# Grid2op/grid2op

Hardware: AMD Instinct MI355X
Metric: env steps/sec (batched DoNothing) (higher is better)
Workload: dtype f64; 1 GPU; l2rpn_case14_sandbox AC Newton-Raphson DoNothing env.step, batch=4096 lanes per GPU; env=l2rpn_case14_sandbox, lanes_per_gpu=4096, total_lanes=4096, env_steps_per_launch=16, observations=every env step -> HBM, cascade=False, kernels=grid-specialised at run time (gpf_jit_enable), parallelism=static lane shards x1, no collective

## Files before the change

grid2op_amd/csrc/gridpf_sparse.hpp:

```cpp
#pragma once
#include <type_traits>
#include "gridpf_common.hpp"

namespace gpf {

struct StatOff {
  int n_dbl, n_int;
  int n_int_hot;
  int br_y, br_bdc, sub_vn_kv, shunt_fact, gen_min_q, gen_max_q;
  int line_vn, load_vn, gen_vn, sto_vn, shunt_vn;
  int line_ka;
  int gen_qmin_tot, gen_qmax_tot;
  int gen_cnt;
  int dc_inv;
  int line_or_pos, line_ex_pos, line_or_sub, line_ex_sub, br_slot, gen_pos, gen_sub, gen_slack, load_pos, load_sub, sto_pos,
      sto_sub, shunt_sub, pair_rc, up, prog;
  int pos_line;
};
#define GPF_STATOFF_INTS(X) X(n_dbl) X(n_int) X(n_int_hot) X(br_y) X(br_bdc) X(sub_vn_kv) X(shunt_fact) X(gen_min_q) X(gen_max_q) X(line_vn) X(load_vn) \
  X(gen_vn) X(sto_vn) X(shunt_vn) X(line_ka) X(gen_qmin_tot) X(gen_qmax_tot) X(gen_cnt) X(dc_inv) X(line_or_pos) X(line_ex_pos) X(line_or_sub) \
  X(line_ex_sub) X(br_slot) X(gen_pos) X(gen_sub) X(gen_slack) X(load_pos) X(load_sub) X(sto_pos) X(sto_sub) X(shunt_sub) X(pair_rc) X(up) X(prog) X(pos_line)
static_assert(sizeof(StatOff) == sizeof(int) * (0 GPF_STATOFF_INTS(GPF_COUNT_FIELD)), "GPF_STATOFF_INTS must list every field of StatOff");
template <class T, bool IN_LDS>
struct SP {
// ... 530 lines not shown
      const double* Al = A + (size_t)(w0 & 0xffffu) * B2 + r * BS;
      const double* bp = rhs + (size_t)p * BS;
      double acc = 0.0;
#pragma unroll
      for (int m = 0; m < BS; ++m) acc = fma(Al[m], bp[m], acc);
      atomicAdd(&rhs[(size_t)(w0 >> 16) * BS + r], -acc);
    }
    GPF_LSYNC();
  }
#ifdef GPF_TIMING
  const long long t_lu1 = __builtin_readcyclecounter();
#endif
  for (int lv = S.n_levels - 1; lv >= 0; --lv) {
    const int ent_off = prog[S.back_off + 2 * lv], n_ent = prog[S.back_off + 2 * lv + 1];
    for (int it = tid; it < n_ent * BS; it += GW) {
      const unsigned w = (unsigned)prog[ent_off + 2 * (it / BS)];
      const int p = prog[ent_off + 2 * (it / BS) + 1], r = it % BS;
      const double* Au = A + (size_t)(w & 0xffffu) * B2 + r * BS;
      const double* xj = rhs + (size_t)(w >> 16) * BS;
      double acc = 0.0;
#pragma unroll
      for (int m = 0; m < BS; ++m) acc = fma(Au[m], xj[m], acc);
      atomicAdd(&rhs[(size_t)p * BS + r], -acc);
    }
    GPF_LSYNC();
  }
#ifdef GPF_TIMING
  if (dbg) { dbg[0] = t_lu1 - t_lu0; dbg[1] = (long long)__builtin_readcyclecounter() - t_lu1; }
#endif
  return ok;
}

constexpr int GPF_WR_CAP_F = 6, GPF_WR_CAP_B = 2;
template <bool ON> struct FlatWords { };
template <> struct FlatWords<true> { unsigned f[2 * GPF_WR_CAP_F], b[2 * GPF_WR_CAP_B]; };
#ifdef GPF_NO_WORDS_RES
template <int NB, int IPW, int WPI> constexpr bool flat_words_ct() { return false; }
#else
template <int NB, int IPW, int WPI> constexpr bool flat_words_ct() { return NB == 1 && IPW > 1 && WPI == 1; }
#endif
__device__ __forceinline__ bool flat_words_fit(const FlatDev& F) { return F.n_fwd <= GPF_WR_CAP_F && F.n_back <= GPF_WR_CAP_B; }
template <int GW, class PP>
__device__ __forceinline__ void flat_words_load(FlatWords<false>&, const FlatDev&, PP, int) {}
template <int GW, class PP>
__device__ __forceinline__ void flat_words_load(FlatWords<true>& W, const FlatDev& F, PP prog, int tid) {
  const bool fit = flat_words_fit(F);
#pragma unroll
  for (int k = 0; k < GPF_WR_CAP_F; ++k) {
    const bool on_f = fit && k < F.n_fwd;
    W.f[2 * k] = on_f ? (unsigned)prog[2 * tid + 2 * GW * k] : 0xffffffffu;
    W.f[2 * k + 1] = on_f ? (unsigned)prog[2 * tid + 2 * GW * k + 1] : 0u;
  }
#pragma unroll
  for (int k = 0; k < GPF_WR_CAP_B; ++k) {
    const bool on_b = fit && k < F.n_back;
    W.b[2 * k] = on_b ? (unsigned)prog[F.back_off + 2 * tid + 2 * GW * k] : 0xffffffffu;
    W.b[2 * k + 1] = on_b ? (unsigned)prog[F.back_off + 2 * tid + 2 * GW * k + 1] : 0u;
  }
}

template <int GW, class PP = const int*, bool RES = false>
__device__ inline bool block_lu_flat(const FlatDev& F, PP prog, double* __restrict__ A, size_t HS, int tid, long long* dbg = nullptr,
                                     const FlatWords<RES>* W = nullptr) {
#ifdef GPF_TIMING
  const long long t_lu0 = __builtin_readcyclecounter();
#endif
  bool ok = true;
#ifdef GPF_PF2_IG
  constexpr bool PF2 = GPF_PF2_ON && (GW > WAVE || (GW <= 32 && !std::is_same<PP, const int*>::value));
#else
  constexpr bool PF2 = GPF_PF2_ON && GW > WAVE;
#endif
  char* const a0 = reinterpret_cast<char*>(A);
  char* const a1 = a0 + HS * 8;
#define FL_LD2(base, f) (*reinterpret_cast<const double2*>((base) + (f)))
#define FL_D(base, f) (reinterpret_cast<double*>((base) + (f)))
#ifdef GPF_TIMING
#define GPF_PASS_T(i_) do { if (dbg && tid == 0 && (i_) < GPF_NPASS_T) gpf_pass_t[(i_)] = (long long)__builtin_readcyclecounter(); } while (0)
#else
#define GPF_PASS_T(i_) do {} while (0)
#endif
  GPF_PASS_T(0);
  auto fwd_item = [&](const unsigned w0, const unsigned w1) {
    if (w0 != 0xffffffffu) {
      const unsigned fd = w0 & 0xffffu, fl = w0 >> 16, fu = w1 & 0xffffu, fp = w1 >> 16;
      const double2 dA = FL_LD2(a0, fp), dB = FL_LD2(a1, fp), lA = FL_LD2(a0, fl), lB = FL_LD2(a1, fl);
      const double2 uA = FL_LD2(a0, fu), uB = FL_LD2(a1, fu);
      const double rd = -fast_rcp(fma(dA.x, dB.y, -dA.y * dB.x));
      const double t00 = fma(lA.x, dB.y, -lA.y * dB.x), t01 = fma(lA.y, dA.x, -lA.x * dA.y);
      const double t10 = fma(lB.x, dB.y, -lB.y * dB.x), t11 = fma(lB.y, dA.x, -lB.x * dA.y);
      double* d0_ = FL_D(a0, fd);
      double* d1_ = FL_D(a1, fd);
      atomicAdd(&d0_[0], fma(t00, uA.x, t01 * uB.x) * rd);
      atomicAdd(&d1_[0], fma(t10, uA.x, t11 * uB.x) * rd);
      if (fd < (unsigned)F.rhs_field0) {
        atomicAdd(&d0_[1], fma(t00, uA.y, t01 * uB.y) * rd);
        atomicAdd(&d1_[1], fma(t10, uA.y, t11 * uB.y) * rd);
      }
    }
  };
#define GPF_WALK(n_, at0_, MASK_, NEXT_SOLO_, ITEM_, TB_, WR_, CAP_)                                                                                 \
  {                                                                                                                                \
    const unsigned solo_ = GW > WAVE ? (unsigned)(MASK_) : 0u;                                                                     \
    const int n_pass_ = (n_);                                                                                                      \
    auto step_ = [&](const unsigned a_, const unsigned b_, const int k) {                                                          \
      const bool so_ = GW > WAVE && k < 32 && ((solo_ >> (k & 31)) & 1u);                                                          \
      if (!so_ || tid < WAVE) ITEM_(a_, b_);                                                                                       \
      const bool sn_ = so_ && (k + 1 < n_pass_ ? (k + 1 < 32 && ((solo_ >> ((k + 1) & 31)) & 1u)) : (GW > WAVE && (NEXT_SOLO_)));  \
      if (sn_) { asm volatile("" ::: "memory"); __builtin_amdgcn_wave_barrier(); asm volatile("" ::: "memory"); }                 \
      else GPF_LSYNC();                                                                                                            \
      GPF_PASS_T((TB_) + k);                                                                                                       \
    };                                                                                                                             \
    if constexpr (RES) {                                   \
      _Pragma("unroll")                                                                                                            \
      for (int k = 0; k < (CAP_); ++k)                                                                                             \
        if (k < n_pass_) step_(W->WR_[2 * k], W->WR_[2 * k + 1], k);                                                               \
    } else {                                                                                                                       \
    int at = (at0_) + 2 * tid;                                                                                                     \
    unsigned p0 = (unsigned)prog[at], p1 = (unsigned)prog[at + 1];                                                                 \
    if (PF2) {                                                                                                                     \
      at += 2 * GW;                                                                                                                \
      unsigned q0 = (unsigned)prog[at], q1 = (unsigned)prog[at + 1], r0, r1;                                                       \
      for (int k = 0; k < n_pass_; k += 3) {                                                                                       \
        at += 2 * GW; r0 = (unsigned)prog[at]; r1 = (unsigned)prog[at + 1];                                                        \
        step_(p0, p1, k);                                                                                                          \
        if (k + 1 >= n_pass_) break;                                                                                               \
        at += 2 * GW; p0 = (unsigned)prog[at]; p1 = (unsigned)prog[at + 1];                                                        \
        step_(q0, q1, k + 1);                                                                                                      \
        if (k + 2 >= n_pass_) break;                                                                                               \
        at += 2 * GW; q0 = (unsigned)prog[at]; q1 = (unsigned)prog[at + 1];                                                        \
        step_(r0, r1, k + 2);                                                                                                      \
      }                                                                                                                            \
    } else {                                                                                                                       \
      for (int k = 0; k < n_pass_; ++k) {                                                                                          \
        at += 2 * GW;                                                                                                              \
        const unsigned n0 = (unsigned)prog[at], n1 = (unsigned)prog[at + 1];                           \
        step_(p0, p1, k);                                                                                                          \
        p0 = n0; p1 = n1;                                                                                                          \
      }                                                                                                                            \
    }                                                                                                                              \
    }                                                                                                                              \
  }
  GPF_WALK(F.n_fwd, 0, F.solo_fwd, F.n_back > 0 && (F.solo_back & 1), fwd_item, 1, f, GPF_WR_CAP_F)
#ifdef GPF_TIMING
  const long long t_lu1 = __builtin_readcyclecounter();
#endif
  auto back_item = [&](const unsigned w0, const unsigned w1) {
    if (w0 != 0xffffffffu) {
      const unsigned fu = w0 & 0xffffu, fj = w0 >> 16, fdj = fj - (unsigned)F.rhs_field0;
      const double2 uA = FL_LD2(a0, fu), uB = FL_LD2(a1, fu), dA = FL_LD2(a0, fdj), dB = FL_LD2(a1, fdj);
      const double s0 = *FL_D(a0, fj), s1 = *FL_D(a1, fj);
      const double rd = fast_rcp(fma(dA.x, dB.y, -dA.y * dB.x));
      const double x0 = fma(dB.y, s0, -dA.y * s1) * rd, x1 = fma(dA.x, s1, -dB.x * s0) * rd;
      atomicAdd(FL_D(a0, w1), -fma(uA.x, x0, uA.y * x1));
      atomicAdd(FL_D(a1, w1), -fma(uB.x, x0, uB.y * x1));
    }
  };
  GPF_WALK(F.n_back, F.back_off, F.solo_back, false, back_item, 1 + F.n_fwd, b, GPF_WR_CAP_B)
#ifdef GPF_TIMING
  if (dbg) { dbg[0] = t_lu1 - t_lu0; dbg[1] = (long long)__builtin_readcyclecounter() - t_lu1; }
#endif
  return ok;
}

template <int GW, bool FACTOR, bool COMPACT, class PP = const int*, bool RES = false>
__device__ inline bool scalar_lu_flat(const FlatDev& F, PP prog, double* __restrict__ A, double* __restrict__ fac, int tid,
                                      long long* dbg = nullptr, const FlatWords<RES>* W = nullptr) {
#ifdef GPF_TIMING
  const long long t_lu0 = __builtin_readcyclecounter();
#endif
  bool ok = true;
#ifdef GPF_PF2_IG
  constexpr bool PF2 = GPF_PF2_ON && (GW > WAVE || (GW <= 32 && !std::is_same<PP, const int*>::value));
#else
  constexpr bool PF2 = GPF_PF2_ON && GW > WAVE;
#endif
  char* const a0 = reinterpret_cast<char*>(A);
  char* const fb = reinterpret_cast<char*>(fac);
  auto facp = [&](unsigned f) -> double* { return reinterpret_cast<double*>(fb + (COMPACT ? (f >> 1) : f)); };
  auto fwd_item = [&](const unsigned w0, const unsigned w1) {
    const unsigned fd = w0 & 0xffffu, fl = w0 >> 16, fu = w1 & 0xffffu, fp = w1 >> 16;
    const bool is_r = (int)fd >= F.rhs_field0;
    if (w0 != 0xffffffffu && (FACTOR || is_r)) {
      const double d = *facp(fp), al = *facp(fl);
      const double x = is_r ? *FL_D(a0, fu) : *facp(fu);
      double* dst = is_r ? FL_D(a0, fd) : facp(fd);
      atomicAdd(dst, -(al * x) * fast_rcp(d));
    }
  };
#undef GPF_PASS_T
#define GPF_PASS_T(i_) do {} while (0)
  GPF_WALK(F.n_fwd, 0, F.solo_fwd, F.n_back > 0 && (F.solo_back & 1), fwd_item, 0, f, GPF_WR_CAP_F)
#ifdef GPF_TIMING
  const long long t_lu1 = __builtin_readcyclecounter();
#endif
  auto back_item = [&](const unsigned w0, const unsigned w1) {
    if (w0 != 0xffffffffu) {
      const unsigned fj = w0 >> 16;
      atomicAdd(FL_D(a0, w1), -(*facp(w0 & 0xffffu) * *FL_D(a0, fj)) * fast_rcp(*facp(fj - (unsigned)F.rhs_field0)));
    }
  };
  GPF_WALK(F.n_back, F.back_off, F.solo_back, false, back_item, 0, b, GPF_WR_CAP_B)
#ifdef GPF_TIMING
  if (dbg) { dbg[0] = t_lu1 - t_lu0; dbg[1] = (long long)__builtin_readcyclecounter() - t_lu1; }
#endif
  return ok;
}
#undef GPF_PASS_T
#undef GPF_WALK
#undef FL_LD2
#undef FL_D

struct SolveCtl {
  bool inj_staged;
  bool topo_staged;
  bool reuse;
  bool dcf;
  bool write_bus;
  bool sums_done;
  bool warm;
  bool otraj;
  int orow;
  bool write_topo;
  bool inj_regs;
  float r_lp0, r_lq0, r_lp1, r_lq1, r_pp, r_vm;
  bool tc_rebuild;
};
struct TopoState {
  int status;
  int nb;
  bool dc_base;
  int dc_out;
  bool gen_base;
  int tc[2];
};

constexpr int YR_PASSES = 4;
template <int NB, int STAGE, int IPW, int WPI, bool TC, bool YR = false>
__device__ inline int solve_instance_sparse(const DevParamsS* __restrict__ P, const SymDev& S, const FlatDev& FL, const StatView<STAGE>& sv, CarveP<NB>& c, double2* yreg, unsigned* rcreg,
                                            const FlatWords<flat_words_ct<NB, IPW, WPI>()>& FW, int inst, int is_dc, int max_iter,
                                            double tol_pu, int tid, const SolveCtl& ctl, TopoState& ts, int& n_iter_out, int& nb_out, float& a_or_first GPF_STAMPS_PARAM) {
  typedef Grp<IPW, WPI> G;
  constexpr int GW = G::GW;
  constexpr int BS = 2 * NB;
  constexpr int B2 = BS * BS;
  GridDev g_loc = P->g;
  GPF_SPEC_G(g_loc);
  pin_sgpr(g_loc.n_sub); pin_sgpr(g_loc.n_line); pin_sgpr(g_loc.n_gen); pin_sgpr(g_loc.n_load); pin_sgpr(g_loc.n_sto);
  pin_sgpr(g_loc.n_shunt); pin_sgpr(g_loc.dim_topo); pin_sgpr(g_loc.nb_tot);
  const GridDev& g = g_loc;
  const Bufs& b = P->b;
#ifdef GPF_JIT
  OutOff oo_loc = P->oo;
  GPF_SPEC_OO(oo_loc);
  const OutOff& oo = oo_loc;
#else
  const OutOff& oo = P->oo;
#endif
  const int nsub = g.n_sub;
  const int nbus = TC ? S.n : nsub * NB;
  constexpr int GWA = WPI > 1 ? WAVE : GW;
  const bool acc_lane = WPI == 1 || tid < WAVE;
  const bool wave1 = WPI > 1 && tid >= WAVE;
  const size_t HS = ((size_t)S.rslot0 + S.n) * 2;
  auto bel = [&](int slot, int r, int col) -> double* {
    return BS == 2 ? c.A + (size_t)r * HS + (size_t)slot * 2 + col : c.A + (size_t)slot * B2 + r * BS + col;
  };
  auto rhsT = [&](int i) -> double* { return BS == 2 ? c.A + ((size_t)S.rslot0 + i) * 2 : c.rhs + (size_t)(i / NB) * BS + 2 * (i % NB); };
  auto rhsV = [&](int i) -> double* { return BS == 2 ? c.A + HS + ((size_t)S.rslot0 + i) * 2 : c.rhs + (size_t)(i / NB) * BS + 2 * (i % NB) + 1; };
  auto SreP = [&](int i) -> double* { return BS == 2 ? c.A + ((size_t)S.rslot0 + i) * 2 + 1 : c.Sre + i; };
  auto SimP = [&](int i) -> double* { return BS == 2 ? c.A + HS + ((size_t)S.rslot0 + i) * 2 + 1 : c.Sim + i; };
  auto EF = [&](int i) -> double2 { return NB == 1 ? reinterpret_cast<const double2*>(c.e)[i] : make_double2(c.e[i], c.f[i]); };
  auto setEF = [&](int i, double e_, double f_) { if (NB == 1) reinterpret_cast<double2*>(c.e)[i] = make_double2(e_, f_); else { c.e[i] = e_; c.f[i] = f_; } };
// ... 255 lines not shown
    }
  }
  GPF_LSYNC();
  if (YR && do_y) {
#pragma unroll
    for (int k = 0; k < YR_PASSES; ++k) {
      const int pr = tid + k * GW;
      const unsigned w0 = pr < S.n_up ? (unsigned)sv.up[2 * pr] : 0u, w1 = pr < S.n_up ? (unsigned)sv.up[2 * pr + 1] : 0u;
      rcreg[2 * k] = w0; rcreg[2 * k + 1] = w1;
      yreg[2 * k] = pr < S.n_up ? *reinterpret_cast<const double2*>(ydst + (size_t)(w1 & 0xffffu) * 2) : make_double2(0.0, 0.0);
      yreg[2 * k + 1] = pr < S.n_up ? *reinterpret_cast<const double2*>(ydst + (size_t)(w1 >> 16) * 2) : make_double2(0.0, 0.0);
    }
    yreg[2 * YR_PASSES] = tid < nbus ? *reinterpret_cast<const double2*>(ydst + (size_t)tid * 2) : make_double2(0.0, 0.0);
    GPF_LSYNC();
  }
  }
  if (!fuse_dc)
  for (int i = tid; i < nbus; i += GW) {
    const int sub = (NB == 1) ? i : i / NB, bi = lidx(i);
    const int bt = c.btype[i];
    const bool th_live = (bt == BT_PQ || bt == BT_PV);
    if (!dc_skip) {
      if (!th_live) *bel(sub, 2 * bi, 2 * bi) = 1.0;
      *bel(sub, 2 * bi + 1, 2 * bi + 1) = 1.0;
    }
    *rhsT(i) = th_live ? (c.Psp[i] - c.Gs[i]) : 0.0;
    *rhsV(i) = 0.0;
  }
  if (!fuse_dc) GPF_LSYNC();
  }
  GPF_STAMPS(3);
  const int* const flat_g = STAGE == 0 ? sv.prog.p : S.flat[gw_index(GW)];
  constexpr bool PROG_LDS = STAGE >= 1 && IPW == 1;
  constexpr bool WRES = flat_words_ct<NB, IPW, WPI>();
  const bool wres = WRES && flat_words_fit(FL);
  auto lu_ac = [&](long long* dbg) -> bool {
    if (BS == 2) {
      if (WRES && wres) return block_lu_flat<GW, decltype(gptr(flat_g)), WRES>(FL, gptr(flat_g), c.A, HS, tid, dbg, &FW);
      if (PROG_LDS) return block_lu_flat<GW>(FL, sv.prog.p, c.A, HS, tid, dbg);
      return block_lu_flat<GW>(FL, gptr(flat_g), c.A, HS, tid, dbg);
    }
    if (STAGE >= 1) return block_lu_solve<BS, GW>(S, sv.prog.p, c.A, c.rhs, tid, dbg);
    return block_lu_solve<BS, GW>(S, gptr(sv.prog.p), c.A, c.rhs, tid, dbg);
  };
  auto lu_dc = [&](long long* dbg) -> bool {
    if (dc_kept) {
      if (WRES && wres) return scalar_lu_flat<GW, false, true, decltype(gptr(flat_g)), WRES>(FL, gptr(flat_g), c.A, c.Adc, tid, dbg, &FW);
      if (PROG_LDS) return scalar_lu_flat<GW, false, true>(FL, sv.prog.p, c.A, c.Adc, tid, dbg);
      return scalar_lu_flat<GW, false, true>(FL, gptr(flat_g), c.A, c.Adc, tid, dbg);
    }
    if (WRES && wres) return scalar_lu_flat<GW, true, false, decltype(gptr(flat_g)), WRES>(FL, gptr(flat_g), c.A, c.A, tid, dbg, &FW);
    if (PROG_LDS) return scalar_lu_flat<GW, true, false>(FL, sv.prog.p, c.A, c.A, tid, dbg);
    return scalar_lu_flat<GW, true, false>(FL, gptr(flat_g), c.A, c.A, tid, dbg);
  };
  if (!warm && !fuse_dc) {
#ifdef GPF_TIMING
    bool ok = dc_inv ? true : (NB == 1) ? lu_dc(&stamps.v[20])
                                        : lu_ac(&stamps.v[20]);
#else
    bool ok = dc_inv ? true : (NB == 1) ? lu_dc(nullptr) : lu_ac(nullptr);
#endif
    for (int i = tid; i < nbus; i += GW) {
      double th;
      if (dc_inv) {
        auto row_times_rhs = [&](const auto tab) -> double {
          double t0 = 0.0, t1 = 0.0;
          for (int k0 = 0; k0 < nbus; k0 += MVC) {
// ... 103 lines not shown
            }
          }
          return t0 + t1;
        };
        const double th = S.so.dc_inv >= 0 ? row_times_rhs(sv.dc_inv, STAGE == 2) : row_times_rhs(sv.dc_inv_g, false);
        const bool live = (bt == BT_PQ || bt == BT_PV);
        va = live ? th : 0.0;
        vm = (vi >= 0 && (bt == BT_PV || bt == BT_REF)) ? GPF_INJ(oo.inj_gen_vm + vi) : vm_lds;
        const bool th_bad = b_on && bt != BT_OFF && !(fabs(th) < 1e300);
        if (status == 0 && G::any(th_bad)) { status = 4; done = true; }
      } else { va = c.va[ib]; vm = c.vm[ib]; }
#ifdef GPF_TIMING
      GPF_STAMPS(21);
#endif
      const bool act = p_on && (btu != BT_OFF) && (btv != BT_OFF);
      const bool uP = (btu == BT_PQ || btu == BT_PV), uQ = (btu == BT_PQ), vP = (btv == BT_PQ || btv == BT_PV), vQ = (btv == BT_PQ);
      const bool acc_u = act && (yuv0.x != 0.0 || yuv0.y != 0.0), acc_v = act && (yvu0.x != 0.0 || yvu0.y != 0.0);
      const bool rowP = (bt == BT_PQ || bt == BT_PV), rowQ = (bt == BT_PQ);
      const bool diag_on = bt != BT_OFF && (ydiag0.x != 0.0 || ydiag0.y != 0.0);
      double* const Ad0 = bel(ib, 0, 0);
      double* const Ad1 = bel(ib, 1, 0);
      double* const b_uv0 = bel(suv, 0, 0); double* const b_uv1 = bel(suv, 1, 0);
      double* const b_vu0 = bel(svu, 0, 0); double* const b_vu1 = bel(svu, 1, 0);
      double e, f, ivm, Sr = 0.0, Si = 0.0;
      {
        double sn_, co;
        fast_sincos(va, sn_, co);
        e = vm * co; f = vm * sn_; ivm = fast_rcp(vm);
        if (b_on) { setEF(ib, e, f); c.ivm[ib] = ivm; *SreP(ib) = 0.0; *SimP(ib) = 0.0; }
      }
      for (int i = S.nslot_y * 2 + tid; i < S.nslot * 2; i += GW) { c.A[i] = 0.0; c.A[HS + i] = 0.0; }
      GPF_LSYNC();
      GPF_STAMPS(10);
      asm volatile("; GPF_NEWTON_NWR_BEGIN" ::: "memory");
      while (true) {
        if (p_on) {
          const double2 efu = EF(u), efv = EF(v);
          const double ivmu = c.ivm[u], ivmv = c.ivm[v];
          double tr_, ti_, sr_, si_;
          const double2 yuv = NWR_YUV, yvu = NWR_YVU;
          t_of(yuv, efu.x, efu.y, efv.x, efv.y, tr_, ti_);
          t_of(yvu, efv.x, efv.y, efu.x, efu.y, sr_, si_);
          *reinterpret_cast<double2*>(b_uv0) = make_double2((uP && vP) ? ti_ : 0.0, (uP && vQ) ? tr_ * ivmv : 0.0);
          *reinterpret_cast<double2*>(b_uv1) = make_double2((uQ && vP) ? -tr_ : 0.0, (uQ && vQ) ? ti_ * ivmv : 0.0);
          *reinterpret_cast<double2*>(b_vu0) = make_double2((vP && uP) ? si_ : 0.0, (vP && uQ) ? sr_ * ivmu : 0.0);
          *reinterpret_cast<double2*>(b_vu1) = make_double2((vQ && uP) ? -sr_ : 0.0, (vQ && uQ) ? si_ * ivmu : 0.0);
          if (acc_u) { atomicAdd(SreP(u), tr_); atomicAdd(SimP(u), ti_); }
          if (acc_v) { atomicAdd(SreP(v), sr_); atomicAdd(SimP(v), si_); }
        }
        GPF_LSYNC();
        if (it == 0) GPF_STAMPS(11);
        double fabs_mis = 0.0;
        bool bad = false;
        if (b_on) {
          Sr = *SreP(ib); Si = *SimP(ib);
          const double2 ydiag = NWR_YD;
          const double psp = NWR_PSP, qsp = NWR_QSP;
          double tr_, ti_;
          t_of(ydiag, e, f, e, f, tr_, ti_);
          if (diag_on) { Sr += tr_; Si += ti_; }
          const double2 r0 = make_double2(rowP ? ti_ : 0.0, (rowP && rowQ) ? tr_ * ivm : 0.0);
          const double2 r1 = make_double2((rowQ && rowP) ? -tr_ : 0.0, rowQ ? ti_ * ivm : 0.0);
          *reinterpret_cast<double2*>(Ad0) = make_double2(rowP ? r0.x - Si : 1.0, rowQ ? fma(Sr, ivm, r0.y) : r0.y);
          *reinterpret_cast<double2*>(Ad1) = make_double2(rowQ ? r1.x + Sr : r1.x, rowQ ? fma(Si, ivm, r1.y) : 1.0);
          const double mp = rowP ? (Sr - psp) : 0.0;
          const double mq = rowQ ? (Si - qsp) : 0.0;
          *rhsT(ib) = -mp; *rhsV(ib) = -mq;
          const double am = fmax(fabs(mp), fabs(mq));
          if (!(am <= 1e300)) bad = true;
          fabs_mis = am;
        }
        if (!done) {
          const unsigned fl = G::template any2<0>(!(fabs_mis < tol_pu), bad);
          if (fl & 2u) { status = 1; done = true; }
          else if (!(fl & 1u)) { converged = true; done = true; }
          else if (it >= max_iter) done = true;
          else ++it;
        }
        if (G::block_all_u(done)) break;
        GPF_LSYNC();
        if (it == 1) GPF_STAMPS(12);
#ifdef GPF_TIMING
        const bool ok = lu_ac(it == 1 ? &stamps.v[32] : nullptr);
#else
        const bool ok = lu_ac(nullptr);
#endif
        if (it == 1) GPF_STAMPS(13);
        bool fin = true, piv_ok = true;
        if (b_on) {
          double2 dx = make_double2(*rhsT(ib), *rhsV(ib));
          const double2 dA = *reinterpret_cast<const double2*>(Ad0), dB = *reinterpret_cast<const double2*>(Ad1);
          const double det = fma(dA.x, dB.y, -dA.y * dB.x);
          if (!(fabs(det) > 1e-300) || !(fabs(det) < 1e300)) piv_ok = false;
          const double rd = fast_rcp(det);
          dx = make_double2(fma(dB.y, dx.x, -dA.y * dx.y) * rd, fma(dA.x, dx.y, -dB.x * dx.x) * rd);
          if (!done && bt != BT_OFF) {
            if (!(fabs(dx.x) < 1e300) || !(fabs(dx.y) < 1e300)) fin = false;
            if (bt == BT_PQ || bt == BT_PV) va += dx.x;
            if (bt == BT_PQ) vm += dx.y;
            if (vm < 0.0) { vm = -vm; va += 3.14159265358979323846; }
            if (fabs(va) > 3.14159265358979323846) va = remainder(va, 6.28318530717958647692);
          }
          double sn_, co;
          fast_sincos(va, sn_, co);
          e = vm * co; f = vm * sn_; ivm = fast_rcp(vm);
          setEF(ib, e, f);
          c.ivm[ib] = ivm;
          *SreP(ib) = 0.0;
          *SimP(ib) = 0.0;
        }
        for (int i = S.nslot_y * 2 + tid; i < S.nslot * 2; i += GW) { c.A[i] = 0.0; c.A[HS + i] = 0.0; }
        GPF_LSYNC();
        if (!done && G::template any2<1>(!ok || !piv_ok, !fin) != 0u) { status = 4; done = true; }
        if (it == 1) GPF_STAMPS(14);
        asm volatile("; GPF_NEWTON_NWR_BACKEDGE" ::: "memory");
      }
      if (b_on) { *SreP(ib) = Sr; *SimP(ib) = Si; c.va[ib] = va; c.vm[ib] = vm; }
#undef NWR_YUV
#undef NWR_YVU
#undef NWR_YD
#undef NWR_PSP
#undef NWR_QSP
    } else {
      for (int i = tid; i < nbus; i += GW) {
        const double va = c.va[i], vmi = c.vm[i];
        double sn_, co;
        fast_sincos(va, sn_, co);
        setEF(i, vmi * co, vmi * sn_);
        if (NB == 1) c.ivm[i] = fast_rcp(vmi);
        *SreP(i) = 0.0;
        *SimP(i) = 0.0;
        if (WPI > 1) { *rhsT(i) = 0.0; *rhsV(i) = 0.0; }
      }
      if (BS == 2) { for (int i = S.nslot_y * 2 + tid; i < S.nslot * 2; i += GW) { c.A[i] = 0.0; c.A[HS + i] = 0.0; } }
      else for (int i = S.nslot_y * B2 + tid; i < S.nslot_lu * B2; i += GW) c.A[i] = 0.0;
      GPF_LSYNC();
      GPF_STAMPS(10);
      unsigned rc_first = 0, rc_first1 = 0;
      if (STAGE == 0 && !YR) {
        if (NB == 1) { if (tid < S.n_up) { rc_first = (unsigned)sv.up[2 * tid]; rc_first1 = (unsigned)sv.up[2 * tid + 1]; } }
        else if (tid < n_pairs) rc_first = (unsigned)sv.pair_rc[tid / (NB * NB)];
      }
      while (true) {
        if (NB == 1) {
          auto upair_item = [&](const unsigned w0, const unsigned w1, const double2 yuv, const double2 yvu) {
            const int u = (int)(w0 & 0xffffu), v = (int)(w0 >> 16), suv = (int)(w1 & 0xffffu), svu = (int)(w1 >> 16);
// ... 501 lines not shown
#ifdef GPF_FORCE_MINW
#define GPF_MINW(m_) GPF_FORCE_MINW
#else
#define GPF_MINW(m_) m_
#endif

template <int NB, int STAGE, int IPW, int MINW, int WPI, bool TC = false, bool YR = false>
__global__ __launch_bounds__(WAVE * WPI, GPF_MINW(MINW)) void runpf_sparse_kernel(const DevParamsS* __restrict__ P, int lane0, const int* __restrict__ lane_list,
                                                            const int* __restrict__ lane_class, int is_dc, int max_iter,
                                                            double tol_pu) {
  extern __shared__ __attribute__((aligned(16))) unsigned char smem[];
  constexpr int GW = Grp<IPW, WPI>::GW;
  const int grp = threadIdx.x / GW, tid = threadIdx.x % GW;
  const int inst = lane_list ? gptr(lane_list)[blockIdx.x * IPW + grp] : lane0 + blockIdx.x * IPW + grp;
  CarveP<NB> c;
#ifdef GPF_JIT
  GridDev g_k = P->g;
  GPF_SPEC_G(g_k);
  const GridDev& g = g_k;
#else
  const GridDev& g = P->g;
#endif
  GPF_CARVE_AND_VIEW(g, P->dcf != 0);
  double2 yreg[2 * YR_PASSES + 1];
  unsigned rcreg[2 * YR_PASSES];
  int n_iter, nb;
  float a_first = 0.f;
  GPF_STAMPS_DECL;
  SolveCtl ctl;
  ctl.inj_staged = false; ctl.topo_staged = false; ctl.reuse = false; ctl.dcf = false; ctl.write_bus = true; ctl.warm = false; ctl.sums_done = false;
  ctl.otraj = false; ctl.orow = inst; ctl.write_topo = true; ctl.inj_regs = false; ctl.tc_rebuild = false;
  TopoState ts;
  ts.status = 0; ts.nb = 0; ts.dc_base = false; ts.dc_out = -1; ts.gen_base = false; ts.tc[0] = ts.tc[1] = -1;
  FlatWords<flat_words_ct<NB, IPW, WPI>()> FW;
  flat_words_load<GW>(FW, FL, gptr(S.flat[GWI]), tid);
  const int st = solve_instance_sparse<NB, STAGE, IPW, WPI, TC, YR>(P, S, FL, sv, c, yreg, rcreg, FW, inst, is_dc, max_iter, tol_pu, tid, ctl, ts, n_iter, nb, a_first GPF_STAMPS_ARG);
  GPF_SYNC();
  if (st != 0) write_nan_results<GW>(g, P->b, inst, tid, inst, false);
  if (tid == 0) {
    const auto s = gptr(P->b.status) + (size_t)inst * 4;
    s[0] = st; s[1] = n_iter; s[2] = nb; s[3] = 0;
  }
}

template <int KIND, int CTRL, int ROW_MASK>
__device__ __forceinline__ double env_dpp_step(double v) {
  const int lo_ = __double2loint(v), hi_ = __double2hiint(v);
  const int lo = __builtin_amdgcn_update_dpp(KIND == 0 ? 0 : lo_, lo_, CTRL, ROW_MASK, 0xF, false);
  const int hi = __builtin_amdgcn_update_dpp(KIND == 0 ? 0 : hi_, hi_, CTRL, ROW_MASK, 0xF, false);
  const double o = __hiloint2double(hi, lo);
  return KIND == 0 ? v + o : KIND == 1 ? fmin(v, o) : fmax(v, o);
}
template <int LW, int KIND>
__device__ __forceinline__ double env_greduce(double v) {
  v = env_dpp_step<KIND, 0xB1, 0xF>(v);
  v = env_dpp_step<KIND, 0x4E, 0xF>(v);
  v = env_dpp_step<KIND, 0x141, 0xF>(v);
  v = env_dpp_step<KIND, 0x140, 0xF>(v);
  if (LW == 16) return v;
  v = env_dpp_step<KIND, 0x142, 0xA>(v);
  if (LW == 32) {
    const double s0 = readlane_f64(v, 31), s1 = readlane_f64(v, 63);
    return (threadIdx.x & 32) ? s1 : s0;
  }
  v = env_dpp_step<KIND, 0x143, 0xC>(v);
  return readlane_f64(v, 63);
}
template <int LW> __device__ __forceinline__ double env_gsum(double v) { return env_greduce<LW, 0>(v); }
// ... 372 lines not shown
      for (int ch = tid + KC * GW; ch < n_ch; ch += GW) put4(ch, km16[ch]);
      if (!YR) {
        double2* const yl = reinterpret_cast<double2*>(c.Yb);
#pragma unroll
        for (int u = 0; u < KY; ++u) { const int i = tid + u * GW; if (i < S.nslot_y) yl[i] = yy[u]; }
        for (int i = tid + KY * GW; i < S.nslot_y; i += GW) { const v2d_ t_ = ky[i]; yl[i] = make_double2(t_.x, t_.y); }
      }
      if (keep_dcf && (k_h2 & 4)) {
#pragma unroll
        for (int u = 0; u < KA; ++u) { const int q = tid + u * GW; if (q < S.nslot) c.Adc[q] = aa[u]; }
        for (int q = tid + KA * GW; q < S.nslot; q += GW) c.Adc[q] = ka[q];
      }
    }
    GPF_STAMPS(37);
    const unsigned hb = G::template any_bits<3, 4>(((same && valid) ? 0u : 1u) | ((k_h2 & 1) ? 0u : 2u) | ((k_h2 & 4) ? 0u : 4u) | (same ? 0u : 8u));
    const unsigned hbb = IPW == 1 ? hb : ((__any(hb & 1u) ? 1u : 0u) | (__any(hb & 2u) ? 2u : 0u) | (__any(hb & 4u) ? 4u : 0u));
    keep_hit = !(hbb & 1u) && (!keep_dcf || !(hbb & 2u) || !(hbb & 4u));
    keep_claim = !(hb & 8u) && k_h0 == KEEP_KEYED && !ghost;
    if (keep_hit) {
      ts.status = k_h1 & 0xff; ts.nb = k_h1 >> 8; ts.dc_base = (k_h2 & 1) != 0; ts.gen_base = (k_h2 & 2) != 0; ts.dc_out = (k_h2 >> 3) - 1;
      reuse = true;
    }
    GPF_STAMPS(38);
    GPF_LSYNC();
  }
  GPF_STAMPS(39);
#define GPF_REDERIVE()                                                                                              \
  do {                                                                                                              \
    grp = grp0; tid = tid0; inst = inst0;                                                                           \
    asm volatile("" : "+v"(grp), "+v"(tid), "+v"(inst));                                                            \
    carve_sparse<NB>(c, smem + (size_t)grp * per_inst, g, lds_nslot, lds_nslot_y, STAGE != 0, lds_rows, lds_dcf);   \
  } while (0)
  const bool tobs = b.traj_out != nullptr;
  FlatWords<flat_words_ct<NB, IPW, WPI>()> FW;
  flat_words_load<GW>(FW, FL, gptr(S.flat[GWI]), tid0);
  for (int step = 0; step < sa.n_steps; ++step) {
    GPF_REDERIVE();
    const bool last = step + 1 == sa.n_steps;
    const bool otraj = tobs && step < b.traj_cap;
    int orow = otraj ? step * (int)b.lane_stride + inst : inst;
    GPF_STAMPS(19);
    bool sums_in_k9 = false, skip_inj = false;
    float k9_lp0 = 0.f, k9_lq0 = 0.f, k9_lp1 = 0.f, k9_lq1 = 0.f, k9_pp = 0.f, k9_vm = 1.f;
    {
      const auto ch = gptr(b.chron) + ((size_t)tab * sa.T + row) * g.n_chron;
      const auto sc = gptr(b.lane_scale) + (size_t)inst * 2 * g.n_load;
      const auto gdelta = gptr(b.lane_gen_delta) + (size_t)inst * g.n_gen;
      const auto inj_g = gptr(b.inj) + (size_t)inst * g.n_inj;
      bool any_maint = false;
      const auto mrow = gptr(b.maint) + ((size_t)tab * sa.T + row) * g.n_line;
      if (b.maint) {
        const auto topo = gptr(b.topo) + (size_t)inst * g.dim_topo;
        bool hit = false;
        if (!ghost)
        for (int l = tid; l < g.n_line; l += GW)
          if (mrow[l] && topo[sv.line_or_pos[l]] != -1) { topo[sv.line_or_pos[l]] = -1; topo[sv.line_ex_pos[l]] = -1; hit = true; }
        any_maint = G::block_any(hit);
        if (any_maint) reuse = false;
      }
      if (!reuse) { const auto topo = gptr(b.topo) + (size_t)inst * g.dim_topo; for (int i = tid; i < g.dim_topo; i += GW) c.topo[i] = topo[i]; }
      if (any_maint) {
        GPF_SYNC();
        for (int l = tid; l < g.n_line; l += GW) if (mrow[l]) { c.topo[sv.line_or_pos[l]] = -1; c.topo[sv.line_ex_pos[l]] = -1; }
      }
      float pp_pre = pf_pp, pv_pre = pf_pv, lp_pre = pf_lp, lq_pre = pf_lq;
      constexpr bool PRE2 = WPI > 1;
      constexpr int gw9 = WPI > 1 ? WAVE : GW;
      float lp2 = 0.f, lq2 = 0.f, sc2p = 1.f, sc2q = 1.f;
// ... 311 lines not shown
```

Before: 218.7 million env steps/sec.

## Pre-resolve LU program words to LDS addresses and defer Jacobian writes past convergence check

Adds a third register-resident word mode (JIT builds with TC off) that decodes the flat LU program once into absolute LDS byte addresses, so each forward and backward elimination item issues direct ds loads and atomics without unpacking offsets. That mode always does a full LDS sync per pass instead of the solo-wave barrier path. In the same mode, Newton Jacobian and RHS stores are held in registers and written only after the convergence check, so the final iteration skips them, and branchy status updates become predicated wave-wide any() reductions. The cost is more live VGPRs (about 30 address words plus ten saved Jacobian terms), which may lower occupancy.

```diff
diff --git a/grid2op_amd/csrc/gridpf_sparse.hpp b/grid2op_amd/csrc/gridpf_sparse.hpp
--- a/grid2op_amd/csrc/gridpf_sparse.hpp
+++ b/grid2op_amd/csrc/gridpf_sparse.hpp
@@ -586,18 +586,28 @@
 }
 
 constexpr int GPF_WR_CAP_F = 6, GPF_WR_CAP_B = 2;
-template <bool ON> struct FlatWords { };
-template <> struct FlatWords<true> { unsigned f[2 * GPF_WR_CAP_F], b[2 * GPF_WR_CAP_B]; };
+typedef __attribute__((address_space(3))) char lds_char;
+typedef __attribute__((address_space(3))) double lds_double;
+typedef double gpf_d2 __attribute__((ext_vector_type(2)));
+typedef __attribute__((address_space(3))) gpf_d2 lds_d2;
+__device__ __forceinline__ unsigned lds_addr(const void* p) { return (unsigned)reinterpret_cast<size_t>((const lds_char*)p); }
+__device__ __forceinline__ lds_char* lds_at(unsigned a) { return reinterpret_cast<lds_char*>((size_t)a); }
+constexpr unsigned GPF_NO_ITEM = 0xffffffffu;
+template <int MODE> struct FlatWords { };
+template <> struct FlatWords<1> { unsigned f[2 * GPF_WR_CAP_F], b[2 * GPF_WR_CAP_B]; };
+template <> struct FlatWords<2> { unsigned f[4 * GPF_WR_CAP_F], b[3 * GPF_WR_CAP_B], base, lim; };
 #ifdef GPF_NO_WORDS_RES
-template <int NB, int IPW, int WPI> constexpr bool flat_words_ct() { return false; }
+template <int NB, int IPW, int WPI, bool TC = true> constexpr int flat_words_ct() { return 0; }
+#elif defined(GPF_JIT)
+template <int NB, int IPW, int WPI, bool TC = true> constexpr int flat_words_ct() { return NB == 1 && IPW > 1 && WPI == 1 ? (TC ? 1 : 2) : 0; }
 #else
-template <int NB, int IPW, int WPI> constexpr bool flat_words_ct() { return NB == 1 && IPW > 1 && WPI == 1; }
+template <int NB, int IPW, int WPI, bool TC = true> constexpr int flat_words_ct() { return NB == 1 && IPW > 1 && WPI == 1 ? 1 : 0; }
 #endif
 __device__ __forceinline__ bool flat_words_fit(const FlatDev& F) { return F.n_fwd <= GPF_WR_CAP_F && F.n_back <= GPF_WR_CAP_B; }
 template <int GW, class PP>
-__device__ __forceinline__ void flat_words_load(FlatWords<false>&, const FlatDev&, PP, int) {}
+__device__ __forceinline__ void flat_words_load(FlatWords<0>&, const FlatDev&, PP, int, const double*) {}
 template <int GW, class PP>
-__device__ __forceinline__ void flat_words_load(FlatWords<true>& W, const FlatDev& F, PP prog, int tid) {
+__device__ __forceinline__ void flat_words_load(FlatWords<1>& W, const FlatDev& F, PP prog, int tid, const double*) {
   const bool fit = flat_words_fit(F);
 #pragma unroll
   for (int k = 0; k < GPF_WR_CAP_F; ++k) {
@@ -612,10 +622,40 @@
     W.b[2 * k + 1] = on_b ? (unsigned)prog[F.back_off + 2 * tid + 2 * GW * k + 1] : 0u;
   }
 }
-
-template <int GW, class PP = const int*, bool RES = false>
+template <int GW, class PP>
+__device__ __forceinline__ void flat_words_load(FlatWords<2>& W, const FlatDev& F, PP prog, int tid, const double* A) {
+  const bool fit = flat_words_fit(F);
+  const unsigned base = lds_addr(A);
+  W.base = base;
+  W.lim = base + (unsigned)F.rhs_field0;
+#pragma unroll
+  for (int k = 0; k < GPF_WR_CAP_F; ++k) {
+    const bool on_f = fit && k < F.n_fwd;
+    const unsigned w0 = on_f ? (unsigned)prog[2 * tid + 2 * GW * k] : 0xffffffffu;
+    const unsigned w1 = on_f ? (unsigned)prog[2 * tid + 2 * GW * k + 1] : 0u;
+    W.f[4 * k] = w0 != 0xffffffffu ? base + (w0 & 0xffffu) : GPF_NO_ITEM;
+    W.f[4 * k + 1] = base + (w0 >> 16);
+    W.f[4 * k + 2] = base + (w1 & 0xffffu);
+    W.f[4 * k + 3] = base + (w1 >> 16);
+  }
+#pragma unroll
+  for (int k = 0; k < GPF_WR_CAP_B; ++k) {
+    const bool on_b = fit && k < F.n_back;
+    const unsigned w0 = on_b ? (unsigned)prog[F.back_off + 2 * tid + 2 * GW * k] : 0xffffffffu;
+    const unsigned w1 = on_b ? (unsigned)prog[F.back_off + 2 * tid + 2 * GW * k + 1] : 0u;
+    W.b[3 * k] = w0 != 0xffffffffu ? base + (w0 & 0xffffu) : GPF_NO_ITEM;
+    W.b[3 * k + 1] = base + (w0 >> 16) - (unsigned)F.rhs_field0;
+    W.b[3 * k + 2] = base + w1;
+  }
+#pragma unroll
+  for (int i = 0; i < 4 * GPF_WR_CAP_F; ++i) asm volatile("" : "+v"(W.f[i]));
+#pragma unroll
+  for (int i = 0; i < 3 * GPF_WR_CAP_B; ++i) asm volatile("" : "+v"(W.b[i]));
+}
+
+template <int GW, class PP = const int*, int RES = 0>
 __device__ inline bool block_lu_flat(const FlatDev& F, PP prog, double* __restrict__ A, size_t HS, int tid, long long* dbg = nullptr,
-                                     const FlatWords<RES>* W = nullptr) {
+                                     FlatWords<RES>* W = nullptr) {
 #ifdef GPF_TIMING
   const long long t_lu0 = __builtin_readcyclecounter();
 #endif
@@ -653,6 +693,37 @@
       }
     }
   };
+  if constexpr (RES == 2) {
+#pragma unroll
+    for (int k = 0; k < GPF_WR_CAP_F; ++k) asm volatile("" : "+v"(W->f[4 * k]));
+#pragma unroll
+    for (int k = 0; k < GPF_WR_CAP_B; ++k) asm volatile("" : "+v"(W->b[3 * k]));
+  }
+  auto fwd_item_res = [&](const int k) {
+    if constexpr (RES == 2) {
+      const unsigned ad = W->f[4 * k];
+      if (ad != GPF_NO_ITEM) {
+        const lds_char* const pp = lds_at(W->f[4 * k + 3]);
+        const lds_char* const pl = lds_at(W->f[4 * k + 1]);
+        const lds_char* const pu = lds_at(W->f[4 * k + 2]);
+        lds_char* const pd = lds_at(ad);
+        const gpf_d2 dA = *reinterpret_cast<const lds_d2*>(pp), dB = *reinterpret_cast<const lds_d2*>(pp + HS * 8);
+        const gpf_d2 lA = *reinterpret_cast<const lds_d2*>(pl), lB = *reinterpret_cast<const lds_d2*>(pl + HS * 8);
+        const gpf_d2 uA = *reinterpret_cast<const lds_d2*>(pu), uB = *reinterpret_cast<const lds_d2*>(pu + HS * 8);
+        const double rd = -fast_rcp(fma(dA.x, dB.y, -dA.y * dB.x));
+        const double t00 = fma(lA.x, dB.y, -lA.y * dB.x), t01 = fma(lA.y, dA.x, -lA.x * dA.y);
+        const double t10 = fma(lB.x, dB.y, -lB.y * dB.x), t11 = fma(lB.y, dA.x, -lB.x * dA.y);
+        double* const d0_ = (double*)reinterpret_cast<lds_double*>(pd);
+        double* const d1_ = (double*)reinterpret_cast<lds_double*>(pd + HS * 8);
+        atomicAdd(&d0_[0], fma(t00, uA.x, t01 * uB.x) * rd);
+        atomicAdd(&d1_[0], fma(t10, uA.x, t11 * uB.x) * rd);
+        if (ad < W->lim) {
+          atomicAdd(&d0_[1], fma(t00, uA.y, t01 * uB.y) * rd);
+          atomicAdd(&d1_[1], fma(t10, uA.y, t11 * uB.y) * rd);
+        }
+      }
+    }
+  };
 #define GPF_WALK(n_, at0_, MASK_, NEXT_SOLO_, ITEM_, TB_, WR_, CAP_)                                                                                 \
   {                                                                                                                                \
     const unsigned solo_ = GW > WAVE ? (unsigned)(MASK_) : 0u;                                                                     \
@@ -665,11 +736,15 @@
       else GPF_LSYNC();                                                                                                            \
       GPF_PASS_T((TB_) + k);                                                                                                       \
     };                                                                                                                             \
-    if constexpr (RES) {                                   \
+    if constexpr (RES == 2) {          \
+      _Pragma("unroll")                                                                                                            \
+      for (int k = 0; k < (CAP_); ++k)                                                                                             \
+        if (k < n_pass_) { ITEM_##_res(k); GPF_LSYNC(); GPF_PASS_T((TB_) + k); }                 \
+    } else if constexpr (RES == 1) {                       \
       _Pragma("unroll")                                                                                                            \
       for (int k = 0; k < (CAP_); ++k)                                                                                             \
         if (k < n_pass_) step_(W->WR_[2 * k], W->WR_[2 * k + 1], k);                                                               \
-    } else {                                                                                                                       \
+    } else {                                                                                                                  \
     int at = (at0_) + 2 * tid;                                                                                                     \
     unsigned p0 = (unsigned)prog[at], p1 = (unsigned)prog[at + 1];                                                                 \
     if (PF2) {                                                                                                                     \
@@ -710,6 +785,24 @@
       atomicAdd(FL_D(a1, w1), -fma(uB.x, x0, uB.y * x1));
     }
   };
+  auto back_item_res = [&](const int k) {
+    if constexpr (RES == 2) {
+      const unsigned au = W->b[3 * k];
+      if (au != GPF_NO_ITEM) {
+        const lds_char* const pu = lds_at(au);
+        const lds_char* const pdj = lds_at(W->b[3 * k + 1]);
+        const lds_char* const pj = pdj + F.rhs_field0;
+        lds_char* const pd = lds_at(W->b[3 * k + 2]);
+        const gpf_d2 uA = *reinterpret_cast<const lds_d2*>(pu), uB = *reinterpret_cast<const lds_d2*>(pu + HS * 8);
+        const gpf_d2 dA = *reinterpret_cast<const lds_d2*>(pdj), dB = *reinterpret_cast<const lds_d2*>(pdj + HS * 8);
+        const double s0 = *reinterpret_cast<const lds_double*>(pj), s1 = *reinterpret_cast<const lds_double*>(pj + HS * 8);
+        const double rd = fast_rcp(fma(dA.x, dB.y, -dA.y * dB.x));
+        const double x0 = fma(dB.y, s0, -dA.y * s1) * rd, x1 = fma(dA.x, s1, -dB.x * s0) * rd;
+        atomicAdd((double*)reinterpret_cast<lds_double*>(pd), -fma(uA.x, x0, uA.y * x1));
+        atomicAdd((double*)reinterpret_cast<lds_double*>(pd + HS * 8), -fma(uB.x, x0, uB.y * x1));
+      }
+    }
+  };
   GPF_WALK(F.n_back, F.back_off, F.solo_back, false, back_item, 1 + F.n_fwd, b, GPF_WR_CAP_B)
 #ifdef GPF_TIMING
   if (dbg) { dbg[0] = t_lu1 - t_lu0; dbg[1] = (long long)__builtin_readcyclecounter() - t_lu1; }
@@ -717,9 +810,9 @@
   return ok;
 }
 
-template <int GW, bool FACTOR, bool COMPACT, class PP = const int*, bool RES = false>
+template <int GW, bool FACTOR, bool COMPACT, class PP = const int*, int RES = 0>
 __device__ inline bool scalar_lu_flat(const FlatDev& F, PP prog, double* __restrict__ A, double* __restrict__ fac, int tid,
-                                      long long* dbg = nullptr, const FlatWords<RES>* W = nullptr) {
+                                      long long* dbg = nullptr, FlatWords<RES>* W = nullptr) {
 #ifdef GPF_TIMING
   const long long t_lu0 = __builtin_readcyclecounter();
 #endif
@@ -742,6 +835,12 @@
       atomicAdd(dst, -(al * x) * fast_rcp(d));
     }
   };
+  auto fwd_item_res = [&](const int k) {
+    if constexpr (RES == 2) {
+      const unsigned ad = W->f[4 * k], bs = W->base;
+      fwd_item(ad != GPF_NO_ITEM ? ((ad - bs) | ((W->f[4 * k + 1] - bs) << 16)) : 0xffffffffu, (W->f[4 * k + 2] - bs) | ((W->f[4 * k + 3] - bs) << 16));
+    }
+  };
 #undef GPF_PASS_T
 #define GPF_PASS_T(i_) do {} while (0)
   GPF_WALK(F.n_fwd, 0, F.solo_fwd, F.n_back > 0 && (F.solo_back & 1), fwd_item, 0, f, GPF_WR_CAP_F)
@@ -752,6 +851,12 @@
     if (w0 != 0xffffffffu) {
       const unsigned fj = w0 >> 16;
       atomicAdd(FL_D(a0, w1), -(*facp(w0 & 0xffffu) * *FL_D(a0, fj)) * fast_rcp(*facp(fj - (unsigned)F.rhs_field0)));
+    }
+  };
+  auto back_item_res = [&](const int k) {
+    if constexpr (RES == 2) {
+      const unsigned au = W->b[3 * k], bs = W->base;
+      back_item(au != GPF_NO_ITEM ? ((au - bs) | ((W->b[3 * k + 1] - bs + (unsigned)F.rhs_field0) << 16)) : 0xffffffffu, W->b[3 * k + 2] - bs);
     }
   };
   GPF_WALK(F.n_back, F.back_off, F.solo_back, false, back_item, 0, b, GPF_WR_CAP_B)
@@ -792,7 +897,7 @@
 constexpr int YR_PASSES = 4;
 template <int NB, int STAGE, int IPW, int WPI, bool TC, bool YR = false>
 __device__ inline int solve_instance_sparse(const DevParamsS* __restrict__ P, const SymDev& S, const FlatDev& FL, const StatView<STAGE>& sv, CarveP<NB>& c, double2* yreg, unsigned* rcreg,
-                                            const FlatWords<flat_words_ct<NB, IPW, WPI>()>& FW, int inst, int is_dc, int max_iter,
+                                            FlatWords<flat_words_ct<NB, IPW, WPI, TC>()>& FW, int inst, int is_dc, int max_iter,
                                             double tol_pu, int tid, const SolveCtl& ctl, TopoState& ts, int& n_iter_out, int& nb_out, float& a_or_first GPF_STAMPS_PARAM) {
   typedef Grp<IPW, WPI> G;
   constexpr int GW = G::GW;
@@ -1114,7 +1219,7 @@
   GPF_STAMPS(3);
   const int* const flat_g = STAGE == 0 ? sv.prog.p : S.flat[gw_index(GW)];
   constexpr bool PROG_LDS = STAGE >= 1 && IPW == 1;
-  constexpr bool WRES = flat_words_ct<NB, IPW, WPI>();
+  constexpr int WRES = flat_words_ct<NB, IPW, WPI, TC>();
   const bool wres = WRES && flat_words_fit(FL);
   auto lu_ac = [&](long long* dbg) -> bool {
     if (BS == 2) {
@@ -1284,6 +1389,12 @@
       for (int i = S.nslot_y * 2 + tid; i < S.nslot * 2; i += GW) { c.A[i] = 0.0; c.A[HS + i] = 0.0; }
       GPF_LSYNC();
       GPF_STAMPS(10);
+#ifdef GPF_NO_LATE_J
+      constexpr bool LATE_J = false;
+#else
+      constexpr bool LATE_J = WRES == 2;
+#endif
+      double j_tr, j_ti, j_sr, j_si, j_ivmu, j_ivmv, j_dtr, j_dti, j_mp, j_mq;
       asm volatile("; GPF_NEWTON_NWR_BEGIN" ::: "memory");
       while (true) {
         if (p_on) {
@@ -1293,10 +1404,12 @@
           const double2 yuv = NWR_YUV, yvu = NWR_YVU;
           t_of(yuv, efu.x, efu.y, efv.x, efv.y, tr_, ti_);
           t_of(yvu, efv.x, efv.y, efu.x, efu.y, sr_, si_);
+          if (!LATE_J) {
           *reinterpret_cast<double2*>(b_uv0) = make_double2((uP && vP) ? ti_ : 0.0, (uP && vQ) ? tr_ * ivmv : 0.0);
           *reinterpret_cast<double2*>(b_uv1) = make_double2((uQ && vP) ? -tr_ : 0.0, (uQ && vQ) ? ti_ * ivmv : 0.0);
           *reinterpret_cast<double2*>(b_vu0) = make_double2((vP && uP) ? si_ : 0.0, (vP && uQ) ? sr_ * ivmu : 0.0);
           *reinterpret_cast<double2*>(b_vu1) = make_double2((vQ && uP) ? -sr_ : 0.0, (vQ && uQ) ? si_ * ivmu : 0.0);
+          } else { j_tr = tr_; j_ti = ti_; j_sr = sr_; j_si = si_; j_ivmu = ivmu; j_ivmv = ivmv; }
           if (acc_u) { atomicAdd(SreP(u), tr_); atomicAdd(SimP(u), ti_); }
           if (acc_v) { atomicAdd(SreP(v), sr_); atomicAdd(SimP(v), si_); }
         }
@@ -1311,18 +1424,29 @@
           double tr_, ti_;
           t_of(ydiag, e, f, e, f, tr_, ti_);
           if (diag_on) { Sr += tr_; Si += ti_; }
+          if (!LATE_J) {
           const double2 r0 = make_double2(rowP ? ti_ : 0.0, (rowP && rowQ) ? tr_ * ivm : 0.0);
           const double2 r1 = make_double2((rowQ && rowP) ? -tr_ : 0.0, rowQ ? ti_ * ivm : 0.0);
           *reinterpret_cast<double2*>(Ad0) = make_double2(rowP ? r0.x - Si : 1.0, rowQ ? fma(Sr, ivm, r0.y) : r0.y);
           *reinterpret_cast<double2*>(Ad1) = make_double2(rowQ ? r1.x + Sr : r1.x, rowQ ? fma(Si, ivm, r1.y) : 1.0);
+          }
           const double mp = rowP ? (Sr - psp) : 0.0;
           const double mq = rowQ ? (Si - qsp) : 0.0;
-          *rhsT(ib) = -mp; *rhsV(ib) = -mq;
+          if (!LATE_J) { *rhsT(ib) = -mp; *rhsV(ib) = -mq; }
+          else { j_dtr = tr_; j_dti = ti_; j_mp = mp; j_mq = mq; }
           const double am = fmax(fabs(mp), fabs(mq));
           if (!(am <= 1e300)) bad = true;
           fabs_mis = am;
         }
-        if (!done) {
+        if (LATE_J) {
+          const bool a_bad = G::any(!(fabs_mis <= 1e300)), a_open = G::any(!(fabs_mis < tol_pu));
+          const bool live = !done, f_bad = live && a_bad, f_conv = live && !a_bad && !a_open, f_more = live && !a_bad && a_open;
+          const bool below = it < max_iter;
+          status = f_bad ? 1 : status;
+          converged = converged || f_conv;
+          done = done || f_bad || f_conv || (f_more && !below);
+          it += (f_more && below) ? 1 : 0;
+        } else if (!done) {
           const unsigned fl = G::template any2<0>(!(fabs_mis < tol_pu), bad);
           if (fl & 2u) { status = 1; done = true; }
           else if (!(fl & 1u)) { converged = true; done = true; }
@@ -1330,6 +1454,21 @@
           else ++it;
         }
         if (G::block_all_u(done)) break;
+        if constexpr (LATE_J) {
+          if (p_on) {
+            *reinterpret_cast<double2*>(b_uv0) = make_double2((uP && vP) ? j_ti : 0.0, (uP && vQ) ? j_tr * j_ivmv : 0.0);
+            *reinterpret_cast<double2*>(b_uv1) = make_double2((uQ && vP) ? -j_tr : 0.0, (uQ && vQ) ? j_ti * j_ivmv : 0.0);
+            *reinterpret_cast<double2*>(b_vu0) = make_double2((vP && uP) ? j_si : 0.0, (vP && uQ) ? j_sr * j_ivmu : 0.0);
+            *reinterpret_cast<double2*>(b_vu1) = make_double2((vQ && uP) ? -j_sr : 0.0, (vQ && uQ) ? j_si * j_ivmu : 0.0);
+          }
+          if (b_on) {
+            const double2 r0 = make_double2(rowP ? j_dti : 0.0, (rowP && rowQ) ? j_dtr * ivm : 0.0);
+            const double2 r1 = make_double2((rowQ && rowP) ? -j_dtr : 0.0, rowQ ? j_dti * ivm : 0.0);
+            *reinterpret_cast<double2*>(Ad0) = make_double2(rowP ? r0.x - Si : 1.0, rowQ ? fma(Sr, ivm, r0.y) : r0.y);
+            *reinterpret_cast<double2*>(Ad1) = make_double2(rowQ ? r1.x + Sr : r1.x, rowQ ? fma(Si, ivm, r1.y) : 1.0);
+            *rhsT(ib) = -j_mp; *rhsV(ib) = -j_mq;
+          }
+        }
         GPF_LSYNC();
         if (it == 1) GPF_STAMPS(12);
 #ifdef GPF_TIMING
@@ -1361,9 +1500,17 @@
           *SreP(ib) = 0.0;
           *SimP(ib) = 0.0;
         }
+        if (LATE_J && (S.nslot - S.nslot_y) * 2 <= GW) {
+          const int i = S.nslot_y * 2 + tid;
+          if (i < S.nslot * 2) { c.A[i] = 0.0; c.A[HS + i] = 0.0; }
+        } else
         for (int i = S.nslot_y * 2 + tid; i < S.nslot * 2; i += GW) { c.A[i] = 0.0; c.A[HS + i] = 0.0; }
         GPF_LSYNC();
-        if (!done && G::template any2<1>(!ok || !piv_ok, !fin) != 0u) { status = 4; done = true; }
+        if (LATE_J) {
+          const bool f_num = !done && G::any(!ok || !piv_ok || !fin);
+          status = f_num ? 4 : status;
+          done = done || f_num;
+        } else if (!done && G::template any2<1>(!ok || !piv_ok, !fin) != 0u) { status = 4; done = true; }
         if (it == 1) GPF_STAMPS(14);
         asm volatile("; GPF_NEWTON_NWR_BACKEDGE" ::: "memory");
       }
@@ -1931,8 +2078,8 @@
   ctl.otraj = false; ctl.orow = inst; ctl.write_topo = true; ctl.inj_regs = false; ctl.tc_rebuild = false;
   TopoState ts;
   ts.status = 0; ts.nb = 0; ts.dc_base = false; ts.dc_out = -1; ts.gen_base = false; ts.tc[0] = ts.tc[1] = -1;
-  FlatWords<flat_words_ct<NB, IPW, WPI>()> FW;
-  flat_words_load<GW>(FW, FL, gptr(S.flat[GWI]), tid);
+  FlatWords<flat_words_ct<NB, IPW, WPI, TC>()> FW;
+  flat_words_load<GW>(FW, FL, gptr(S.flat[GWI]), tid, c.A);
   const int st = solve_instance_sparse<NB, STAGE, IPW, WPI, TC, YR>(P, S, FL, sv, c, yreg, rcreg, FW, inst, is_dc, max_iter, tol_pu, tid, ctl, ts, n_iter, nb, a_first GPF_STAMPS_ARG);
   GPF_SYNC();
   if (st != 0) write_nan_results<GW>(g, P->b, inst, tid, inst, false);
@@ -2371,8 +2518,8 @@
     carve_sparse<NB>(c, smem + (size_t)grp * per_inst, g, lds_nslot, lds_nslot_y, STAGE != 0, lds_rows, lds_dcf);   \
   } while (0)
   const bool tobs = b.traj_out != nullptr;
-  FlatWords<flat_words_ct<NB, IPW, WPI>()> FW;
-  flat_words_load<GW>(FW, FL, gptr(S.flat[GWI]), tid0);
+  FlatWords<flat_words_ct<NB, IPW, WPI, TC>()> FW;
+  flat_words_load<GW>(FW, FL, gptr(S.flat[GWI]), tid0, c.A);
   for (int step = 0; step < sa.n_steps; ++step) {
     GPF_REDERIVE();
     const bool last = step + 1 == sa.n_steps;
```

After: 226.8 million env steps/sec, median of 6. 3.7% higher.
